# hherlyng/knp-emi-cgx

Measured on AMD Instinct MI355X. Metric: MDoF/s per implicit timestep (assembly+GMRES), higher is better.
Workload: dtype f64

## Files before the change

### include/knpemi_hip.h

```cpp
#ifndef KNPEMI_HIP_H
#define KNPEMI_HIP_H

#include <stdint.h>

#ifdef __cplusplus
extern "C" {
#endif

#define KNP_MAX_IONS 3
#define KNP_MAX_AUX 8
#define KNP_DIAG_MAX_CONSTS 64
#define KNP_MAX_PROG_REGS 48
#define KNP_MAX_AMG_LEVELS 16

#define KNP_OK 0
#define KNP_E_ARG (-1)
#define KNP_E_HIP (-2)
#define KNP_E_STATE (-3)
#define KNP_E_ALLOC (-4)
#define KNP_E_MESH (-5)

#define KNP_CONVERGED_RTOL 2
#define KNP_CONVERGED_ATOL 3
#define KNP_DIVERGED_ITS (-3)
// ... 105 lines not shown
int knp_matrix_max_abs(knp_ctx* ctx, double* out );

int knp_set_params(knp_ctx* ctx, double dt, double F, double C_M, double psi, int32_t n_ions,
                   const double* z, const double* Di, const double* De);
int knp_set_program(knp_ctx* ctx, int32_t prog_id, int32_t n_instr, const int32_t* code ,
                    int32_t n_consts, const double* consts );
const char* knp_jit_status(knp_ctx* ctx);
int knp_jit_compile_check(const int32_t* code, int32_t n_instr, const char* arch, char* log, int32_t log_cap);
int knp_host_thread_count(void);
int knp_set_program_constants(knp_ctx* ctx, int32_t prog_id, int32_t n_consts, const double* consts);
int knp_set_dirichlet(knp_ctx* ctx, int32_t n, const int32_t* dofs);
int knp_set_sources(knp_ctx* ctx, const double* const* f_i, const double* const* f_e);

int knp_assemble_matrix(knp_ctx* ctx, const knp_fields* fields);
int knp_assemble_matrix_async(knp_ctx* ctx, const knp_fields* fields);
int knp_assemble_rhs(knp_ctx* ctx, const knp_fields* fields, double* b );
int knp_assemble_precond(knp_ctx* ctx, const knp_fields* fields);
int knp_pc_set_coupled_potential(knp_ctx* ctx, int32_t on);
int knp_get_precond_phi_csr(const knp_ctx* ctx, int32_t* rowptr, int32_t* colind, double* vals);

int knp_spmv(knp_ctx* ctx, const double* x, double* y);
int knp_set_nullspace(knp_ctx* ctx, int32_t on);
int knp_project_nullspace(knp_ctx* ctx, double* v);
int knp_nullspace_test(knp_ctx* ctx, double* out_norm );
int knp_pc_setup(knp_ctx* ctx, int32_t kind);
int knp_pc_apply(knp_ctx* ctx, const double* r, double* z);
int knp_set_deflation(knp_ctx* ctx, int32_t n_modes, const int32_t* node_mode, const double* einv);
int knp_amg_reset(knp_ctx* ctx, int32_t hier, int32_t n_levels, int32_t pre_sweeps, int32_t post_sweeps, int32_t cheby_degree);
int knp_amg_set_node_fields(knp_ctx* ctx, int32_t hier, int32_t nf);
int knp_amg_set_level(knp_ctx* ctx, int32_t hier, int32_t level, int32_t n_rows, int32_t n_cols_halo,
// ... 80 lines not shown
```

### knp-emi-cgx_amd/cgx_hip/_lib.py

```python
from __future__ import annotations

import ctypes as C
import os

_HERE = os.path.dirname(os.path.abspath(__file__))
LIB_PATH = os.path.join(_HERE, "libknpemi_hip.so")

KNP_MAX_IONS = 3
KNP_MAX_AUX = 8
KNP_MAX_PROG_REGS = 48
KNP_DIAG_MAX_CONSTS = 64
KNP_SZ_COUNT = 16
(SZ_N_NODES, SZ_N_NODES_OWNED, SZ_N_DOF_LOCAL, SZ_N_DOF_OWNED, SZ_NNZ, SZ_N_PAIRS, SZ_N_CONTRIB,
 SZ_N_GAMMA_VERTS, SZ_N_GAMMA_PAIRS, SZ_NNZ_P, SZ_N_PHI_OWNED, SZ_NNZ_P_PHI, SZ_EMI_NNZ) = range(13)

PC_NONE, PC_VBJACOBI, PC_AMG, PC_AMG_BT, PC_AMG_LT = 0, 1, 2, 3, 4

OPS = dict(CONST=0, KI=1, KE=2, PHIM=3, AUX=4, X=5, ADD=6, SUB=7, MUL=8, DIV=9, NEG=10, POW=11, LN=12,
           EXP=13, SQRT=14, MAX=15, MIN=16, ABS=17, LT=18, GT=19, LE=20, GE=21, EQ=22, AND=23, OR=24,
           NOT=25, SEL=26, OUT=27, MOV=28, POWI=29)

REASONS = {2: "CONVERGED_RTOL", 3: "CONVERGED_ATOL", -3: "DIVERGED_ITS", -4: "DIVERGED_DTOL",
           -9: "DIVERGED_NANORINF", 0: "ITERATING"}

# ... 51 lines not shown
    "knp_set_nullspace": (C.c_int, [vp, C.c_int32]),
    "knp_project_nullspace": (C.c_int, [vp, vp]),
    "knp_nullspace_test": (C.c_int, [vp, f64p]),
    "knp_pc_setup": (C.c_int, [vp, C.c_int32]),
    "knp_pc_apply": (C.c_int, [vp, vp, vp]),
    "knp_set_deflation": (C.c_int, [vp, C.c_int32, i32p, f64p]),
    "knp_amg_reset": (C.c_int, [vp, C.c_int32, C.c_int32, C.c_int32, C.c_int32, C.c_int32]),
    "knp_amg_set_level": (C.c_int, [vp, C.c_int32, C.c_int32, C.c_int32, C.c_int32, i32p, i32p, f64p, f64p, C.c_double,
                                    C.c_int32, i32p, i32p, f64p, i32p, i32p, f64p]),
    "knp_amg_set_level_mode": (C.c_int, [vp, C.c_int32, C.c_int32, C.c_int32, C.c_int32]),
    "knp_amg_set_level_prolongator": (C.c_int, [vp, C.c_int32, C.c_int32, C.c_int32, C.POINTER(C.c_int32), C.POINTER(C.c_int32),
                                               C.POINTER(C.c_double)]),
    "knp_amg_set_coarse": (C.c_int, [vp, C.c_int32, C.c_int32, f64p]),
    "knp_amg_set_level_smoothed": (C.c_int, [vp, C.c_int32, C.c_int32, C.c_int32, i32p, i32p, f64p]),
    "knp_amg_set_level_coarse_fused": (C.c_int, [vp, C.c_int32, C.c_int32, C.c_int32, i32p, i32p, f64p, C.c_int32, i32p, i32p, f64p]),
    "knp_amg_set_node_fields": (C.c_int, [vp, C.c_int32, C.c_int32]),
    "knp_amg_use_native_level0": (C.c_int, [vp, C.c_int32, C.c_int32]),
    "knp_amg_set_precision": (C.c_int, [vp, C.c_int32]),
    "knp_jit_status": (C.c_char_p, [vp]),
    "knp_gmres_prepare": (C.c_int, [vp, vp]),
    "knp_jit_compile_check": (C.c_int, [C.POINTER(C.c_int32), C.c_int32, C.c_char_p, C.c_char_p, C.c_int32]),
    "knp_host_thread_count": (C.c_int, []),
    "knp_p2p_init": (C.c_int, [vp, C.c_int32, C.c_int32, C.c_double]),
    "knp_p2p_shutdown": (C.c_int, [vp]),
    "knp_p2p_plan_create": (C.c_int, [vp, C.c_int32, C.c_int64, C.c_int64, C.POINTER(C.c_int32), vp]),
    "knp_p2p_plan_connect": (C.c_int, [vp, C.c_int32, vp, C.c_int32, C.POINTER(C.c_int32), C.POINTER(C.c_int64),
                                      C.POINTER(C.c_int32), C.POINTER(C.c_int64), C.POINTER(C.c_int64), C.POINTER(C.c_int32),
                                      C.POINTER(C.c_int64)]),
    "knp_p2p_attach": (C.c_int, [vp, C.c_int32, C.c_int32, C.c_int32, C.c_int32]),
    "knp_p2p_test_halo": (C.c_int, [vp, C.c_int32, vp, C.c_int32]),
# ... 65 lines not shown
```

### knp-emi-cgx_amd/cgx_hip/backend.py

```python
from __future__ import annotations

import ctypes as C
import os

import numpy as np
import torch

from . import _lib
from ._lib import Fields, FieldsOut, KnpError, MeshDesc
from .parallel import HaloPlan, all_reduce_sum_, guarded


class _CAI:

    def __init__(self, ptr, n):
        self.__cuda_array_interface__ = {"shape": (int(n),), "typestr": "<f8", "data": (int(ptr), False),
                                         "version": 2, "strides": None}


def _f64(a):
    return a.ctypes.data_as(_lib.f64p)


def _i32(a):
# ... 373 lines not shown
            f.k_e[j] = p.wh[1][j].data_ptr()
        f.phi_i = p.wh[0][3].data_ptr()
        f.phi_e = p.wh[1][3].data_ptr()
        f.phi_m = p.phi_m_prev.data_ptr()
        self._fields_out_cache = f
        return f

    def assemble_matrix(self):
        f = self.fields()
        self.check(self.lib.knp_assemble_matrix(self.ctx, C.byref(f)))

    def assemble_matrix_async(self):
        f = self.fields()
        self.check(self.lib.knp_assemble_matrix_async(self.ctx, C.byref(f)))

    def assemble_rhs(self):
        if not getattr(self, "_programs_uploaded", False):
            self.upload_programs()
        self.refresh_program_constants()
        f = self.fields()
        self.check(self.lib.knp_assemble_rhs(self.ctx, C.byref(f), C.c_void_p(self.b.data_ptr())))

    def assemble_precond(self):
        f = self.fields()
        self.check(self.lib.knp_assemble_precond(self.ctx, C.byref(f)))

    def pack(self):
        f = self.fields_out()
        self.check(self.lib.knp_pack(self.ctx, C.byref(f), C.c_void_p(self.x.data_ptr())))

# ... 245 lines not shown
```

### knp-emi-cgx_amd/cgx_hip/problem.py

```python
from __future__ import annotations

import collections.abc
import ctypes as C
import math
import os
import pathlib
import time
from abc import ABC, abstractmethod

import numpy as np
import torch
import yaml

from . import _lib, fem
from . import mesh as meshmod
from .fem import Constant, Function, FunctionSpace
from .parallel import Comm, LocalMesh, partition_mesh


def range_constructor(loader, node):
    args = loader.construct_sequence(node)
    return list(range(*args))


# ... 533 lines not shown
            self.backend.set_sources()

    def set_initial_conditions(self):
        if self.MMS_test:
            self.print("Setting initial conditions for MMS test ...")
            dev = self.mesh.device
            as_t = lambda a: torch.as_tensor(np.array(a, dtype=np.float64, copy=True), device=dev)
            self.phi_m_prev = Function(self.V, "phi_m")
            self.phi_m_prev.x.array[:] = as_t(self._exact_nodal(self.phi_m_init))
            self.wh[0][self.N_ions].x.array[:] = as_t(self._exact_nodal(self.phi_i_init))
            self.wh[1][self.N_ions].x.array[:] = as_t(self._exact_nodal(self.phi_e_init))
            for idx, ion in enumerate(self.ion_list):
                self.wh[0][idx].x.array[:] = as_t(self._exact_nodal(ion["ki_init"]))
                self.wh[1][idx].x.array[:] = as_t(self._exact_nodal(ion["ke_init"]))
            self.print("Initial conditions set.")
            return
        if self.find_initial_conditions:
            self.find_steady_state_initial_conditions()
        else:
            self.print("Setting initial conditions from input file ...")
        ic = self.initial_conditions
        if not self.glia_flag:
            self.phi_m_init.value = ic["phi_m"] if "phi_m" in ic else ic["phi_m_n"]
            self.Na_i_init.value = ic["Na_i"] if "Na_i" in ic else ic["Na_i_n"]
            self.Na_e_init.value = ic["Na_e"]
            self.K_i_init.value = ic["K_i"] if "K_i" in ic else ic["K_i_n"]
            self.K_e_init.value = ic["K_e"]
            self.Cl_i_init.value = ic["Cl_i"] if "Cl_i" in ic else ic["Cl_i_n"]
            self.Cl_e_init.value = ic["Cl_e"]
        else:
# ... 21 lines not shown
            self.phi_m_prev.x.array[self.glia_dofs] = self.phi_m_g_init.value
            ui_p[self.N_ions].x.array[self.neuron_dofs] = self.phi_m_n_init.value
            ui_p[self.N_ions].x.array[self.glia_dofs] = self.phi_m_g_init.value
            ue_p[self.N_ions].x.array[:] = 0.0
        for idx, ion in enumerate(self.ion_list):
            if self.glia_flag:
                ui_p[idx].x.array[self.neuron_dofs] = ion["ki_init_n"].value
                ui_p[idx].x.array[self.glia_dofs] = ion["ki_init_g"].value
                ue_p[idx].x.array[:] = ion["ke_init"].value
            else:
                ui_p[idx].x.array[:] = ion["ki_init"].value
                ue_p[idx].x.array[:] = ion["ke_init"].value
                self.print(f"Initial condition for {ion['name']}_i set to {ion['ki_init'].value}")
                self.print(f"Initial condition for {ion['name']}_e set to {ion['ke_init'].value}")
        self.print("Initial conditions set.")

    def find_steady_state_initial_conditions(self):
        from .membrane_odes import ThreeCompartmentMembraneODESystem, TwoCompartmentMembraneODESystem
        self.print("Solving ODE system to find steady-state initial conditions ...")
        tic = time.perf_counter()
        self.calculate_compartment_volumes_and_surface_areas()
        areas = (self.area_g_n, self.area_g_g) if self.glia_flag else (self.area_g_n,)
        if not min(areas) > 0:
            raise RuntimeError("Steady-state initial conditions: no membrane facet carries a neuron" + (" or glia" if self.glia_flag else "")
                               + " tag (membrane tags must be the cell tags); provide 'initial_conditions' in the input file.")
        cls = ThreeCompartmentMembraneODESystem if self.glia_flag else TwoCompartmentMembraneODESystem
        odes = cls(self, plot_show=False, plot_save=False, stimulus_flag=False)
        state = None
        if self.comm.rank == 0:
            try:
# ... 199 lines not shown
```

### knp-emi-cgx_amd/cgx_hip/solver.py

```python
from __future__ import annotations

import time

import numpy as np
import torch

import os

from . import _lib, amg, dist_amg
from .ionic_models import HodgkinHuxley
from .problem import ProblemKNPEMI


class _KSPInfo:

    def __init__(self):
        self.its = 0
        self.reason = 0
        self.rnorm = 0.0

    def getIterationNumber(self):
        return self.its

    def getConvergedReason(self):
# ... 315 lines not shown
        be.set_nullspace(True)
        be.project_nullspace(be.b)
        self.print("Null space set.")

    def _matrix_scale(self):
        return self.comm.allreduce_max(self.backend.matrix_max_abs()) + 1e-300

    def _sync(self):
        torch.cuda.synchronize()

    def prepare(self):
        p = self.problem
        self.setup_breakdown = {}
        tic = time.perf_counter()
        self.setup_solver()
        self._sync()
        self.setup_breakdown["solver_setup_s"] = self.comm.allreduce_max(time.perf_counter() - tic)
        self._setup_timer = self.setup_breakdown["solver_setup_s"]
        if self.use_P_mat and self._pc_kind in (_lib.PC_AMG, _lib.PC_AMG_BT, _lib.PC_AMG_LT):
            tic = time.perf_counter()
            p.setup_preconditioner(self.use_block_Jacobi)
            self.assemble_preconditioner()
            self._sync()
            self.setup_breakdown["preconditioner_setup_s"] = self.comm.allreduce_max(time.perf_counter() - tic)
            self._setup_timer += self.setup_breakdown["preconditioner_setup_s"]
        self._n_marked = 0
        self._prepared = True

    def _resolve_timers(self):
        if not getattr(self, "_n_marked", 0):
# ... 184 lines not shown
```

### knp-emi-cgx_amd/csrc/knp_internal.hpp

```cpp
#pragma once
#include <hip/hip_runtime.h>

#include <cstdint>
#include <string>
#include <vector>

#include "knpemi_hip.h"

#define KNP_NPROF 5

struct KnpHostGraph {
    int dim = 0, nv1 = 0;
    int n_v = 0, n_v_owned = 0, n_c = 0, n_c_owned = 0, n_g = 0, n_q = 0;
    int n_nodes = 0, n_nodes_owned = 0;
    std::vector<int32_t> node_i, node_e;
    std::vector<int32_t> node_vertex;
    std::vector<uint8_t> node_side;
    std::vector<int32_t> pair_ptr;
    std::vector<int32_t> pair_col;
    std::vector<int32_t> pair_row;
    std::vector<double> pair_M, pair_K;
    std::vector<int32_t> contrib_ptr;
    std::vector<int32_t> contrib_cell;
    std::vector<double> contrib_k;
// ... 289 lines not shown
    int p2p_red = -1;
    bool hook_allreduce() const { return allreduce && p2p_red < 0; }
    int comm_rc = 0;
    int n_int = 0, n_bnd = 0;
    int32_t *d_nodes_int = nullptr, *d_nodes_bnd = nullptr;
    hipStream_t stream3 = nullptr;
    hipEvent_t ev_x = nullptr, ev_halo = nullptr;
    hipStream_t stream2 = nullptr;
    hipEvent_t ev_fork = nullptr, ev_join = nullptr;
    KnpSidePrep prep;
    bool side_ws = false;
    double *d_t2_s = nullptr, *d_w2_s = nullptr, *d_wb = nullptr, *d_partial_s = nullptr;
    hipStream_t stream_asm = nullptr;
    hipEvent_t ev_fork_asm = nullptr, ev_asm = nullptr;
    bool asm_pending = false;
    double last_bnorm = 0.0;
    int64_t n_allreduce = 0, n_halo = 0, n_readback = 0;
    int64_t n_fused_dots = 0;
    int64_t n_spmv_dots = 0;
    std::vector<hipEvent_t> tm_events;
    size_t tm_used = 0;
    KnpDiagMap diag_cells, diag_facets;
    KnpDiagMap diag_flux;
    double2* d_flux_rec = nullptr;
    KnpDiagMap diag_phim;
    int32_t* diag_code = nullptr;
    int diag_n_instr = 0, diag_n_regs = 0, diag_n_consts = 0;
    double diag_consts[KNP_DIAG_MAX_CONSTS] = {};
    bool diag_prog = false;
    KnpEmi emi;
// ... 10 lines not shown
```

### knp-emi-cgx_amd/csrc/knp_kernels.hip

```cpp
#include <hip/hip_runtime.h>
#include <hip/hip_ext.h>

#include <algorithm>
#include <cmath>
#include <cstdio>
#include <cstdlib>
#include <cstring>
#include <new>

#include "knp_internal.hpp"

#define HIPCHK(call)                                                                       \
    do {                                                                                   \
        hipError_t e_ = (call);                                                            \
        if (e_ != hipSuccess) {                                                            \
            ctx->err = std::string(#call) + ": " + hipGetErrorString(e_);                  \
            return KNP_E_HIP;                                                              \
        }                                                                                  \
    } while (0)
#define KCHK(expr)                         \
    do {                                   \
        int rc_ = (expr);                  \
        if (rc_ != KNP_OK) return rc_;     \
    } while (0)
// ... 13 lines not shown
    double dz2i[3], dz2e[3];
    double rFz[3], cmFz[3];
    double rF;
};
struct FieldPtrs {
    const double* ki[3];
    const double* ke[3];
    const double* phim;
    const double* aux[KNP_MAX_AUX];
};

static void side_discard(knp_ctx* ctx);
static DevParams make_params(const knp_ctx* ctx);
static int64_t phi_block_nnz(const knp_ctx* ctx);
static int join_asm(knp_ctx* ctx);
static bool fin_ok(const knp_ctx* ctx);
static hipEvent_t prof_event(knp_ctx* ctx);
static void free_hier(KnpAmgHier& H);
static inline int nblocks(int64_t n, int per = NT) { return (int)std::max<int64_t>(1, (n + per - 1) / per); }

__device__ __forceinline__ double wave_sum(double v) {
#pragma unroll
    for (int o = 32; o > 0; o >>= 1) v += __shfl_xor(v, o, 64);
    return v;
}
__device__ __forceinline__ double block_sum(double v, double* sm) {
    v = wave_sum(v);
    const int w = threadIdx.x >> 6, l = threadIdx.x & 63;
    __syncthreads();
    if (l == 0) sm[w] = v;
// ... 317 lines not shown
        T0 += __shfl_xor(T0, o, G);
        T1 += __shfl_xor(T1, o, G);
        T2 += __shfl_xor(T2, o, G);
    }
    if (live && selfq < 255 && (selfq & (G - 1)) == lane) emit(p0 + selfq, -T0, -T1, -T2);
}

static void launch_cell_means(knp_ctx* ctx, const FieldPtrs& f) {
    const KnpHostGraph& g = ctx->g;
    if (ctx->asm_dmax > 0)
        hipLaunchKernelGGL(k_nodal_conc, dim3(nblocks(g.n_nodes)), dim3(NT), 0, ctx->stream, g.n_nodes, ctx->d_node_vertex, ctx->d_node_side, f, ctx->d_knod);
    else
        hipLaunchKernelGGL(k_cell_means, dim3(nblocks(g.n_c)), dim3(NT), 0, ctx->stream, g.n_c, g.nv1, ctx->d_cells, ctx->d_cell_side, f, ctx->d_cbar);
}
template <bool PRECOND, bool TD_ONLY>
static void launch_assemble_nodes(knp_ctx* ctx, const DevParams& P, double* at, double* ac) {
    const KnpHostGraph& g = ctx->g;
    const int n = g.n_nodes_owned;
    if (n <= 0) return;
    if (ctx->asm_stage > 0 && ctx->d_tc_meta) {
        const int cmax = ctx->asm_stage;
        const int dmax = ctx->asm_dmax, nv1 = g.nv1;
#define KNP_ASMT2(GG, FF) hipLaunchKernelGGL((k_assemble_nodes_tr<PRECOND, TD_ONLY, GG, FF>), dim3(nblocks((int64_t)n * GG)), dim3(NT),                  \
                                        (size_t)(NT / GG) * (cmax + dmax) * 3 * sizeof(double), ctx->stream, n, P, cmax, ctx->d_pair_ptr, ctx->d_node_side, \
                                        ctx->d_pair_M, ctx->d_pair_K, ctx->d_tc_meta, ctx->d_tc_slot, ctx->d_tc_k, ctx->d_node_cell_ptr,              \
                                        ctx->d_node_cell, ctx->d_cbar, at, ac, ctx->d_pair_col, ctx->d_ncv, ctx->d_knod, dmax, nv1)
#define KNP_ASMT(GG) do { if (dmax > 0) KNP_ASMT2(GG, true); else KNP_ASMT2(GG, false); } while (0)
        switch (ctx->asm_group) {
            case 4: KNP_ASMT(4); break;
            case 8: KNP_ASMT(8); break;
            case 16: KNP_ASMT(16); break;
            default: KNP_ASMT(32); break;
        }
#undef KNP_ASMT
#undef KNP_ASMT2
        return;
    }
    if (ctx->asm_stage > 0) {
        const int cmax = ctx->asm_stage;
        const int dmax = ctx->asm_dmax, nv1 = g.nv1;
#define KNP_ASMS2(GG, FF) hipLaunchKernelGGL((k_assemble_nodes_staged<PRECOND, TD_ONLY, GG, FF>), dim3(nblocks((int64_t)n * GG)), dim3(NT),              \
                                        (size_t)(NT / GG) * (cmax + dmax) * 3 * sizeof(double), ctx->stream, n, P, cmax, ctx->d_pair_ptr, ctx->d_pair_col,  \
                                        ctx->d_node_side, ctx->d_pair_M, ctx->d_pair_K, ctx->d_contrib_ptr, ctx->d_contrib_slot, ctx->d_contrib_k, \
                                        ctx->d_node_cell_ptr, ctx->d_node_cell, ctx->d_cbar, at, ac, ctx->d_ncv, ctx->d_knod, dmax, nv1)
#define KNP_ASMS(GG) do { if (dmax > 0) KNP_ASMS2(GG, true); else KNP_ASMS2(GG, false); } while (0)
        switch (ctx->asm_group) {
            case 4: KNP_ASMS(4); break;
            case 8: KNP_ASMS(8); break;
            case 16: KNP_ASMS(16); break;
            default: KNP_ASMS(32); break;
        }
#undef KNP_ASMS
#undef KNP_ASMS2
        return;
    }
#define KNP_ASM(GG) hipLaunchKernelGGL((k_assemble_nodes<PRECOND, TD_ONLY, GG>), dim3(nblocks((int64_t)n * GG)), dim3(NT), 0, ctx->stream, n, P, ctx->d_pair_ptr, \
                                       ctx->d_pair_col, ctx->d_node_side, ctx->d_pair_M, ctx->d_pair_K, ctx->d_contrib_ptr, ctx->d_contrib_cell,       \
                                       ctx->d_contrib_k, ctx->d_cbar, at, ac)
    switch (ctx->asm_group) {
// ... 2379 lines not shown
    dev_free(ctx->d_V); dev_free(ctx->d_Z); dev_free(ctx->d_w); dev_free(ctx->d_t);
    for (auto& p : ctx->progs) { dev_free(p.d_code); dev_free(p.d_consts); if (p.h_consts) (void)hipHostFree(p.h_consts); }
    dev_free(ctx->d_prog_code); dev_free(ctx->d_prog_consts); dev_free(ctx->d_prog_len); dev_free(ctx->d_prog_nconsts);
    for (int h = 0; h < KNP_MAX_HIER; ++h) free_hier(ctx->hier[h]);
    dev_free(ctx->d_p_vals_f);
    dev_free(ctx->d_ML); dev_free(ctx->d_cc); dev_free(ctx->d_t2); dev_free(ctx->d_w2);
    dev_free(ctx->d_defl_mode); dev_free(ctx->d_defl_einv); dev_free(ctx->d_bc_dofs);
    knp_diag_free(ctx);
    knp_emi_free(ctx);
    delete ctx;
    return KNP_OK;
}

int knp_set_stream(knp_ctx* ctx, void* s) {
    CHECK_CTX(ctx);
    ctx->stream = (hipStream_t)s;
    return KNP_OK;
}
int knp_set_comm(knp_ctx* ctx, knp_halo_fn halo, knp_allreduce_fn ar, void* user) {
    CHECK_CTX(ctx);
    ctx->halo = halo; ctx->allreduce = ar; ctx->comm_user = user;
    ctx->phi_count_cached = -1;
    return KNP_OK;
}

int knp_get_sizes(const knp_ctx* ctx, int64_t* s) {
    if (!ctx || !s) return KNP_E_ARG;
    for (int i = 0; i < KNP_SZ_COUNT; ++i) s[i] = 0;
    s[KNP_SZ_N_NODES] = ctx->g.n_nodes;
    s[KNP_SZ_N_NODES_OWNED] = ctx->g.n_nodes_owned;
// ... 90 lines not shown
    HIPCHK(hipStreamSynchronize(ctx->stream));
    HIPCHK(hipMemcpy(h.data(), ctx->d_partial, h.size() * sizeof(double), hipMemcpyDeviceToHost));
    double m = 0.0;
    for (int k = 0; k < 3; ++k)
        if (len[k] > 0)
            for (int b = 0; b < RED_BLOCKS; ++b) m = std::max(m, h[(size_t)k * RED_BLOCKS + b]);
    *out = m;
    return KNP_OK;
}

int knp_set_params(knp_ctx* ctx, double dt, double F, double C_M, double psi, int32_t n_ions, const double* z,
                   const double* Di, const double* De) {
    CHECK_CTX(ctx);
    if (n_ions != 3 || !z || !Di || !De) { ctx->err = "n_ions must be 3 (Na, K, Cl; KNPEMIx_problem.py:980-981)"; return KNP_E_ARG; }
    if (!(dt > 0) || !(psi > 0) || F == 0.0) { ctx->err = "dt, psi must be positive and F non-zero"; return KNP_E_ARG; }
    ctx->dt = dt; ctx->F = F; ctx->C_M = C_M; ctx->psi = psi; ctx->n_ions = 3;
    ctx->asm_dt = -1.0;
    for (int j = 0; j < 3; ++j) {
        if (z[j] == 0.0 || !(Di[j] > 0) || !(De[j] > 0)) { ctx->err = "valence must be non-zero and diffusivities positive"; return KNP_E_ARG; }
        ctx->z[j] = z[j]; ctx->Di[j] = Di[j]; ctx->De[j] = De[j];
    }
    return KNP_OK;
}

static int validate_program(knp_ctx* ctx, int n_instr, const int32_t* code, int n_consts, int* n_regs_out) {
    int max_reg = -1;
    for (int i = 0; i < n_instr; ++i) {
        const int op = code[4 * i], d = code[4 * i + 1], a = code[4 * i + 2], b = code[4 * i + 3];
        auto regok = [&](int r) { if (r > max_reg) max_reg = r; return r >= 0 && r < KNP_MAX_PROG_REGS; };
        bool ok = true;
// ... 7 lines not shown
            case KNP_OP_MOV: case KNP_OP_POWI: ok = regok(d) && regok(a); break;
            case KNP_OP_OUT: ok = a >= 0 && a < 3 && regok(b); break;
            default: ok = (op >= KNP_OP_ADD && op <= KNP_OP_SEL) && regok(d) && regok(a) && regok(b); break;
        }
        if (!ok) { ctx->err = "invalid membrane program instruction " + std::to_string(i); return KNP_E_ARG; }
    }
    *n_regs_out = max_reg + 1;
    return KNP_OK;
}

int knp_set_program(knp_ctx* ctx, int32_t id, int32_t n_instr, const int32_t* code, int32_t n_consts, const double* consts) {
    CHECK_CTX(ctx);
    if (id < 0 || id > 4096 || n_instr < 0 || (n_instr && !code) || n_consts < 0 || (n_consts && !consts)) { ctx->err = "bad program arguments"; return KNP_E_ARG; }
    int n_regs = 0;
    KCHK(validate_program(ctx, n_instr, code, n_consts, &n_regs));
    if ((int)ctx->progs.size() <= id) ctx->progs.resize(id + 1);
    KnpProgram& p = ctx->progs[id];
    p.n_regs = n_regs;
    HIPCHK(hipStreamSynchronize(ctx->stream));
    dev_free(p.d_code); dev_free(p.d_consts);
    if (p.h_consts) { (void)hipHostFree(p.h_consts); p.h_consts = nullptr; }
    p.n_instr = n_instr; p.n_consts = n_consts;
    p.h_code.assign(code, code + (size_t)4 * n_instr);
    KCHK(dev_upload_raw(ctx, &p.d_code, code, (size_t)4 * n_instr));
    KCHK(dev_upload_raw(ctx, &p.d_consts, consts, (size_t)n_consts));
    ctx->progs_dirty = true;
    return KNP_OK;
}
int knp_set_program_constants(knp_ctx* ctx, int32_t id, int32_t n_consts, const double* consts) {
    CHECK_CTX(ctx);
// ... 28 lines not shown
    KCHK(dev_upload(ctx, &ctx->d_prog_nconsts, ncs));
    ctx->progs_dirty = false;
    knp_jit_build(ctx);
    return KNP_OK;
}

const char* knp_jit_status(knp_ctx* ctx) {
    if (!ctx) return "";
    if (ctx->progs_dirty && !ctx->progs.empty()) (void)sync_program_table(ctx);
    return ctx->jit_msg.c_str();
}

int knp_set_dirichlet(knp_ctx* ctx, int32_t n, const int32_t* dofs) {
    CHECK_CTX(ctx);
    side_discard(ctx);
    if (n < 0 || (n > 0 && !dofs)) { ctx->err = "bad Dirichlet arguments"; return KNP_E_ARG; }
    for (int i = 0; i < n; ++i)
        if (dofs[i] < 0 || dofs[i] >= ctx->n_dof_owned) { ctx->err = "Dirichlet dof out of range (owned dofs only)"; return KNP_E_ARG; }
    HIPCHK(hipStreamSynchronize(ctx->stream));
    dev_free(ctx->d_bc_dofs);
    ctx->n_bc = 0;
    if (n > 0) {
        KCHK(dev_upload_raw(ctx, &ctx->d_bc_dofs, dofs, (size_t)n));
        ctx->n_bc = n;
    }
    ctx->asm_dt = -1.0;
    return KNP_OK;
}

int knp_set_sources(knp_ctx* ctx, const double* const* fi, const double* const* fe) {
// ... 20 lines not shown
    if (ctx->pc_kind == KNP_PC_AMG || ctx->pc_kind == KNP_PC_VBJACOBI) { ctx->have_cc = false; return; }
    const KnpHostGraph& g = ctx->g;
    hipLaunchKernelGGL(k_schur_diag, dim3(nblocks(g.n_nodes_owned)), dim3(NT), 0, ctx->stream, g.n_nodes_owned, ctx->psi, ctx->z[0], ctx->z[1],
                       ctx->z[2], ctx->d_node_vertex, ctx->d_node_side, f, ctx->d_ML, ctx->d_cc);
    ctx->have_cc = true;
}

static int join_asm(knp_ctx* ctx) {
    if (ctx->asm_pending) {
        HIPCHK(hipStreamWaitEvent(ctx->stream, ctx->ev_asm, 0));
        ctx->asm_pending = false;
    }
    return KNP_OK;
}

static int assemble_matrix_on_stream(knp_ctx* ctx, const knp_fields* fields, bool with_schur_diag) {
    const KnpHostGraph& g = ctx->g;
    const DevParams P = make_params(ctx);
    FieldPtrs f = make_fields(fields);
    ProfScope ps(ctx, 3);
    launch_cell_means(ctx, f);
    const bool td_only = ctx->have_A && !ctx->asm_full && ctx->asm_dt == ctx->dt;
    if (td_only) launch_assemble_nodes<false, true>(ctx, P, ctx->d_at, ctx->d_ac);
    else launch_assemble_nodes<false, false>(ctx, P, ctx->d_at, ctx->d_ac);
    ctx->asm_dt = ctx->dt;
    if (g.n_g > 0) {
        if (g.dim == 2)
            hipLaunchKernelGGL((k_gamma_facets<2, true, false, 8, 1, NT, 1>), dim3(nblocks((int64_t)g.n_g * 8)), dim3(NT), 0, ctx->stream, g.n_g, g.n_q, P,
                               ctx->d_fv, ctx->d_fmeas, ctx->d_qp, ctx->d_qw, f, 0, ctx->d_coords, ctx->d_gamma_prog,
                               (const int32_t* const*)nullptr, (const int32_t*)nullptr, (const double* const*)nullptr,
                               (const int32_t*)nullptr, 0, 0, ctx->d_fmat, ctx->d_fvec);
        else if (gamma_many(g)) {
            hipLaunchKernelGGL((k_gamma_facets<3, true, false, 4, 9, 64, 1>), dim3((unsigned)(((int64_t)g.n_g * 4 + 63) / 64)), dim3(64), 0, ctx->stream, g.n_g, g.n_q, P,
                               ctx->d_fv, ctx->d_fmeas, ctx->d_qp, ctx->d_qw, f, 0, ctx->d_coords, ctx->d_gamma_prog,
                               (const int32_t* const*)nullptr, (const int32_t*)nullptr, (const double* const*)nullptr,
                               (const int32_t*)nullptr, 0, 0, ctx->d_fmat, ctx->d_fvec);
        }
        else
            hipLaunchKernelGGL((k_gamma_facets<3, true, false, 16, 3, 64, 2>), dim3((unsigned)(((int64_t)g.n_g * 16 + 63) / 64)), dim3(64), 0, ctx->stream, g.n_g, g.n_q, P,
// ... 12 lines not shown
    if (with_schur_diag && !ctx->prep.left()) launch_schur_diag(ctx, f);
    HIPCHK(hipGetLastError());
    ctx->have_A = true;
    if (ctx->pc_kind == KNP_PC_VBJACOBI) {
        hipLaunchKernelGGL(k_vbj_extract, dim3(nblocks(g.n_nodes_owned)), dim3(NT), 0, ctx->stream, g.n_nodes_owned,
                           ctx->d_pair_ptr, ctx->d_pair_col, ctx->d_ac, ctx->d_at, ctx->d_ax, ctx->d_node_gv, ctx->d_node_side,
                           ctx->d_gdiag, ctx->d_vbj);
        HIPCHK(hipGetLastError());
    }
    return KNP_OK;
}

int knp_assemble_matrix(knp_ctx* ctx, const knp_fields* fields) {
    CHECK_CTX(ctx);
    KCHK(check_fields(ctx, fields, false));
    KCHK(join_asm(ctx));
    return assemble_matrix_on_stream(ctx, fields, true);
}

int knp_assemble_matrix_async(knp_ctx* ctx, const knp_fields* fields) {
    CHECK_CTX(ctx);
    KCHK(check_fields(ctx, fields, false));
    KCHK(join_asm(ctx));
    static const bool off = getenv("KNP_ASM_ASYNC") && atoi(getenv("KNP_ASM_ASYNC")) == 0;
    if (off || ctx->pc_kind == KNP_PC_VBJACOBI || (ctx->prof_on & ~1) || !ctx->have_A || ctx->prep.left())
        return assemble_matrix_on_stream(ctx, fields, true);
    if (!ctx->stream_asm) {
        HIPCHK(hipStreamCreateWithFlags(&ctx->stream_asm, hipStreamNonBlocking));
        HIPCHK(hipEventCreateWithFlags(&ctx->ev_fork_asm, hipEventDisableTiming));
        HIPCHK(hipEventCreateWithFlags(&ctx->ev_asm, hipEventDisableTiming));
    }
    HIPCHK(hipEventRecord(ctx->ev_fork_asm, ctx->stream));
    HIPCHK(hipStreamWaitEvent(ctx->stream_asm, ctx->ev_fork_asm, 0));
    hipStream_t main_stream = ctx->stream;
    ctx->stream = ctx->stream_asm;
    const int rc = assemble_matrix_on_stream(ctx, fields, false);
    ctx->stream = main_stream;
    KCHK(rc);
    HIPCHK(hipEventRecord(ctx->ev_asm, ctx->stream_asm));
    ctx->asm_pending = true;
    return KNP_OK;
}

int knp_pc_set_coupled_potential(knp_ctx* ctx, int32_t on) {
    CHECK_CTX(ctx);
    side_discard(ctx);
    ctx->pc_coupled_phi = on ? 1 : 0;
    if (on && !ctx->d_px) {
        HIPCHK(hipMalloc((void**)&ctx->d_px, (size_t)std::max<int64_t>(ctx->n_gp, 1) * sizeof(double)));
        HIPCHK(hipMemset(ctx->d_px, 0, (size_t)std::max<int64_t>(ctx->n_gp, 1) * sizeof(double)));
    }
    ctx->have_P = false;
    return KNP_OK;
}
static int64_t phi_block_nnz(const knp_ctx* ctx) {
// ... 218 lines not shown
    KCHK(rc);
    if (cnt <= 0) return KNP_OK;
    const int no = ctx->g.n_nodes_owned;
    const int nb = std::min(RED_BLOCKS, nblocks(no));
    hipLaunchKernelGGL(k_phi_sum, dim3(nb), dim3(NT), 0, ctx->stream, no, v, ctx->d_partial);
    hipLaunchKernelGGL(k_reduce_partials, dim3(1), dim3(NT), 0, ctx->stream, nb, ctx->d_partial, ctx->d_red, 62, (double*)nullptr);
    KCHK(allreduce_slots(ctx, 62, 1));
    hipLaunchKernelGGL(k_phi_sub, dim3(nblocks(no)), dim3(NT), 0, ctx->stream, no, ctx->d_red + 62, 1.0 / (double)cnt, v);
    HIPCHK(hipGetLastError());
    return KNP_OK;
}
int knp_project_nullspace(knp_ctx* ctx, double* v) {
    CHECK_CTX(ctx);
    side_discard(ctx);
    if (!v) return KNP_E_ARG;
    return project_ns(ctx, v);
}

static int ensure_work(knp_ctx* ctx, int restart) {
    if (!ctx->d_w) {
        HIPCHK(hipMalloc((void**)&ctx->d_w, std::max(ctx->n_dof_local, 1) * sizeof(double)));
        HIPCHK(hipMalloc((void**)&ctx->d_t, std::max(ctx->n_dof_local, 1) * sizeof(double)));
        HIPCHK(hipMemset(ctx->d_w, 0, std::max(ctx->n_dof_local, 1) * sizeof(double)));
        HIPCHK(hipMemset(ctx->d_t, 0, std::max(ctx->n_dof_local, 1) * sizeof(double)));
    }
    if (restart > 0 && (ctx->gm_restart < restart || !ctx->d_V)) {
        HIPCHK(hipStreamSynchronize(ctx->stream));
        dev_free(ctx->d_V);
        size_t bytes = (size_t)(restart + 1) * std::max(ctx->n_dof_local, 1) * sizeof(double);
        HIPCHK(hipMalloc((void**)&ctx->d_V, bytes));
// ... 998 lines not shown
    if (n_modes == 0) return KNP_OK;
    const int no = ctx->g.n_nodes_owned;
    for (int n = 0; n < no; ++n)
        if (node_mode[n] < -1 || node_mode[n] >= n_modes) { ctx->err = "deflation mode id out of range"; return KNP_E_ARG; }
    dev_free(ctx->d_defl_mode);
    KCHK(dev_upload_raw(ctx, &ctx->d_defl_mode, node_mode, (size_t)no));
    HIPCHK(hipMemcpy(ctx->d_defl_einv, einv, (size_t)n_modes * n_modes * sizeof(double), hipMemcpyHostToDevice));
    ctx->defl_m = n_modes;
    return KNP_OK;
}

int knp_pc_apply(knp_ctx* ctx, const double* r, double* z) {
    CHECK_CTX(ctx);
    side_discard(ctx);
    if (!r || !z) return KNP_E_ARG;
    int rc;
    const int64_t cnt = ctx->ns_on ? global_phi_count(ctx, &rc) : 0;
    return pc_apply_proj(ctx, r, z, cnt);
}

#include "knp_krylov.inc"

static int out_ptrs(knp_ctx* ctx, const knp_fields_out* f, OutPtrs& o, bool need_phim) {
    if (!f) { ctx->err = "null fields"; return KNP_E_ARG; }
    for (int j = 0; j < 3; ++j) {
        if (!f->k_i[j] || !f->k_e[j]) { ctx->err = "null concentration field"; return KNP_E_ARG; }
        o.ki[j] = f->k_i[j]; o.ke[j] = f->k_e[j];
    }
    if (!f->phi_i || !f->phi_e || (need_phim && !f->phi_m)) { ctx->err = "null potential field"; return KNP_E_ARG; }
    o.phi_i = f->phi_i; o.phi_e = f->phi_e; o.phi_m = f->phi_m;
    return KNP_OK;
}
int knp_pack(knp_ctx* ctx, const knp_fields_out* f, double* x) {
    CHECK_CTX(ctx);
    if (!x) return KNP_E_ARG;
    OutPtrs o;
    KCHK(out_ptrs(ctx, f, o, false));
    hipLaunchKernelGGL(k_pack, dim3(nblocks(ctx->g.n_nodes)), dim3(NT), 0, ctx->stream, ctx->g.n_nodes, ctx->d_node_vertex,
                       ctx->d_node_side, o, x);
    HIPCHK(hipGetLastError());
    return KNP_OK;
}
int knp_unpack(knp_ctx* ctx, const double* x, const knp_fields_out* f) {
    CHECK_CTX(ctx);
    if (!x) return KNP_E_ARG;
    OutPtrs o;
    KCHK(out_ptrs(ctx, f, o, true));
    KCHK(join_asm(ctx));
    KCHK(halo_update(ctx, const_cast<double*>(x)));
    hipLaunchKernelGGL(k_unpack, dim3(nblocks(ctx->g.n_v)), dim3(NT), 0, ctx->stream, ctx->g.n_v, ctx->d_node_i, ctx->d_node_e, x, o);
    HIPCHK(hipGetLastError());
    return KNP_OK;
}
int knp_hh_update(knp_ctx* ctx, const double* phi_m, double* n, double* m, double* h, int32_t count, double dt, double phi_rest,
                  int32_t rush_larsen, int32_t substeps) {
    CHECK_CTX(ctx);
    if (!phi_m || !n || !m || !h || count < 0 || substeps < 1 || !(dt > 0)) { ctx->err = "bad hh_update arguments"; return KNP_E_ARG; }
    if (count == 0) return KNP_OK;
    ProfScope ps(ctx, 4);
    hipLaunchKernelGGL(k_hh_update, dim3(nblocks(count)), dim3(NT), 0, ctx->stream, count, phi_m, n, m, h, dt, phi_rest,
                       rush_larsen, substeps);
    HIPCHK(hipGetLastError());
    return KNP_OK;
}
int knp_l2_norms(knp_ctx* ctx, const double* phi_i, const double* phi_e, double* out) {
    CHECK_CTX(ctx);
// ... 143 lines not shown
```

### knp-emi-cgx_amd/csrc/knp_krylov.inc

```

static constexpr int GM_RES = 100, GM_EXPL = 57, GM_MAX_RESTART = GM_EXPL - 2;
static constexpr int FB_SLOT = 124;
static_assert(GM_RES + 2 <= RED_SLOTS && DEFL_SLOT0 + DEFL_MAX <= GM_RES, "reduction slot layout");
static constexpr double GM_DTOL = 1e5;

static void side_discard(knp_ctx* ctx) {
    switch (ctx->prep.kind) {
        case KnpSidePrep::NONE:
        case KnpSidePrep::LEFT_DEFERRED: break;
        default: (void)hipEventSynchronize(ctx->ev_join);
    }
    ctx->prep.kind = KnpSidePrep::NONE;
}
static int ensure_side_stream(knp_ctx* ctx) {
    if (ctx->stream2) return KNP_OK;
    HIPCHK(hipStreamCreateWithFlags(&ctx->stream2, hipStreamNonBlocking));
    HIPCHK(hipEventCreateWithFlags(&ctx->ev_fork, hipEventDisableTiming));
    HIPCHK(hipEventCreateWithFlags(&ctx->ev_join, hipEventDisableTiming));
    return KNP_OK;
}

static bool exchanges_all_native(const knp_ctx* ctx) {
    if (!ctx->p2p || ctx->p2p_fine < 0 || ctx->p2p_red < 0 || ctx->defl_m > 0) return false;
    const int nh = ctx->pc_kind == KNP_PC_AMG ? 1 : (ctx->pc_kind == KNP_PC_AMG_BT || ctx->pc_kind == KNP_PC_AMG_LT) ? 2 : 0;
// ... 182 lines not shown
    knp_ctx* ctx;
    GmLayout GL;
    double* gm;
    int n;
    int64_t ldv;
    int nb, vec_blocks;
    bool ns;
    double inv_cnt;
    double ttol, atol, dref;
};

static int krylov_begin(knp_ctx* ctx, const double* b, double* x, int32_t max_it, int32_t restart, int32_t* its, double* rnorm, int32_t* reason,
                        bool flexible, KrylovSolve* K, int64_t* cnt) {
    if (!b || !x || !its || !rnorm || !reason) return KNP_E_ARG;
    if (!ctx->have_A) { ctx->err = "matrix not assembled"; return KNP_E_STATE; }
    if (restart < 1 || restart > GM_MAX_RESTART || max_it < 0) {
        ctx->err = "restart must be in [1," + std::to_string(GM_MAX_RESTART) + "] and max_it >= 0";
        return KNP_E_ARG;
    }
    KCHK(ensure_work(ctx, restart));
    if (flexible && ctx->pc_kind != KNP_PC_NONE) KCHK(ensure_z(ctx, restart));
    prof_collect_ready(ctx);
    int rc;
    *cnt = ctx->ns_on ? global_phi_count(ctx, &rc) : 0;
    if (ctx->ns_on) KCHK(rc);
    const GmLayout GL{restart};
    if (ctx->gm_cap < GL.size()) {
        HIPCHK(hipStreamSynchronize(ctx->stream));
        dev_free(ctx->d_gm);
        HIPCHK(hipMalloc((void**)&ctx->d_gm, (size_t)GL.size() * sizeof(double)));
// ... 315 lines not shown
```

Before: 2194.

## Prefetch next-step matrix assembly on side stream right after solution unpack

After unpacking the solution into field arrays, the matrix assembly for the next timestep is launched immediately on the separate assembly stream, using the solution vector directly as nodal concentrations instead of recomputing cell means. A later async-assemble call with the same field pointers and dt becomes a no-op and is counted as a prefetch hit. Guards join the assembly stream before anything writes the solution vector, and the prefetch is invalidated whenever params, programs, Dirichlet data, the stream or initial conditions change. This hides assembly latency behind host work between steps, at the cost of extra invalidation logic and a risk of stale-data bugs if a field write is missed.

```diff
diff --git a/include/knpemi_hip.h b/include/knpemi_hip.h
--- a/include/knpemi_hip.h
+++ b/include/knpemi_hip.h
@@ -143,6 +143,9 @@
 
 int knp_assemble_matrix(knp_ctx* ctx, const knp_fields* fields);
 int knp_assemble_matrix_async(knp_ctx* ctx, const knp_fields* fields);
+int knp_set_assembly_prefetch(knp_ctx* ctx, int32_t on);
+int knp_invalidate_fields(knp_ctx* ctx);
+int knp_get_assembly_prefetch_hits(knp_ctx* ctx, int64_t* out);
 int knp_assemble_rhs(knp_ctx* ctx, const knp_fields* fields, double* b );
 int knp_assemble_precond(knp_ctx* ctx, const knp_fields* fields);
 int knp_pc_set_coupled_potential(knp_ctx* ctx, int32_t on);
diff --git a/knp-emi-cgx_amd/cgx_hip/_lib.py b/knp-emi-cgx_amd/cgx_hip/_lib.py
--- a/knp-emi-cgx_amd/cgx_hip/_lib.py
+++ b/knp-emi-cgx_amd/cgx_hip/_lib.py
@@ -89,6 +89,9 @@
     "knp_amg_set_coarse": (C.c_int, [vp, C.c_int32, C.c_int32, f64p]),
     "knp_amg_set_level_smoothed": (C.c_int, [vp, C.c_int32, C.c_int32, C.c_int32, i32p, i32p, f64p]),
     "knp_amg_set_level_coarse_fused": (C.c_int, [vp, C.c_int32, C.c_int32, C.c_int32, i32p, i32p, f64p, C.c_int32, i32p, i32p, f64p]),
+    "knp_set_assembly_prefetch": (C.c_int, [vp, C.c_int32]),
+    "knp_invalidate_fields": (C.c_int, [vp]),
+    "knp_get_assembly_prefetch_hits": (C.c_int, [vp, C.POINTER(C.c_int64)]),
     "knp_amg_set_node_fields": (C.c_int, [vp, C.c_int32, C.c_int32]),
     "knp_amg_use_native_level0": (C.c_int, [vp, C.c_int32, C.c_int32]),
     "knp_amg_set_precision": (C.c_int, [vp, C.c_int32]),
diff --git a/knp-emi-cgx_amd/cgx_hip/backend.py b/knp-emi-cgx_amd/cgx_hip/backend.py
--- a/knp-emi-cgx_amd/cgx_hip/backend.py
+++ b/knp-emi-cgx_amd/cgx_hip/backend.py
@@ -411,6 +411,19 @@
         f = self.fields()
         self.check(self.lib.knp_assemble_matrix_async(self.ctx, C.byref(f)))
 
+    def set_assembly_prefetch(self, on=True):
+        self.check(self.lib.knp_set_assembly_prefetch(self.ctx, 1 if on else 0))
+
+    def invalidate_fields(self):
+        self._fields_cache = None
+        self._fields_out_cache = None
+        self.check(self.lib.knp_invalidate_fields(self.ctx))
+
+    def assembly_prefetch_hits(self):
+        out = C.c_int64()
+        self.check(self.lib.knp_get_assembly_prefetch_hits(self.ctx, C.byref(out)))
+        return out.value
+
     def assemble_rhs(self):
         if not getattr(self, "_programs_uploaded", False):
             self.upload_programs()
diff --git a/knp-emi-cgx_amd/cgx_hip/problem.py b/knp-emi-cgx_amd/cgx_hip/problem.py
--- a/knp-emi-cgx_amd/cgx_hip/problem.py
+++ b/knp-emi-cgx_amd/cgx_hip/problem.py
@@ -571,6 +571,7 @@
                 self.wh[0][idx].x.array[:] = as_t(self._exact_nodal(ion["ki_init"]))
                 self.wh[1][idx].x.array[:] = as_t(self._exact_nodal(ion["ke_init"]))
             self.print("Initial conditions set.")
+            self._fields_rewritten()
             return
         if self.find_initial_conditions:
             self.find_steady_state_initial_conditions()
@@ -622,6 +623,12 @@
                 self.print(f"Initial condition for {ion['name']}_i set to {ion['ki_init'].value}")
                 self.print(f"Initial condition for {ion['name']}_e set to {ion['ke_init'].value}")
         self.print("Initial conditions set.")
+        self._fields_rewritten()
+
+    def _fields_rewritten(self):
+        be = getattr(self, "backend", None)
+        if be is not None and getattr(be, "ctx", None):
+            be.invalidate_fields()
 
     def find_steady_state_initial_conditions(self):
         from .membrane_odes import ThreeCompartmentMembraneODESystem, TwoCompartmentMembraneODESystem
diff --git a/knp-emi-cgx_amd/cgx_hip/solver.py b/knp-emi-cgx_amd/cgx_hip/solver.py
--- a/knp-emi-cgx_amd/cgx_hip/solver.py
+++ b/knp-emi-cgx_amd/cgx_hip/solver.py
@@ -353,6 +353,7 @@
         self.setup_breakdown = {}
         tic = time.perf_counter()
         self.setup_solver()
+        self.backend.set_assembly_prefetch(not p.MMS_test)
         self._sync()
         self.setup_breakdown["solver_setup_s"] = self.comm.allreduce_max(time.perf_counter() - tic)
         self._setup_timer = self.setup_breakdown["solver_setup_s"]
diff --git a/knp-emi-cgx_amd/csrc/knp_internal.hpp b/knp-emi-cgx_amd/csrc/knp_internal.hpp
--- a/knp-emi-cgx_amd/csrc/knp_internal.hpp
+++ b/knp-emi-cgx_amd/csrc/knp_internal.hpp
@@ -327,6 +327,16 @@
     hipStream_t stream_asm = nullptr;
     hipEvent_t ev_fork_asm = nullptr, ev_asm = nullptr;
     bool asm_pending = false;
+    int asm_prefetch = 0;
+    struct KnpPrefetch {
+        bool valid = false;
+        const double* ki[3] = {nullptr, nullptr, nullptr};
+        const double* ke[3] = {nullptr, nullptr, nullptr};
+        const double* phim = nullptr;
+        const double* x = nullptr;
+        double dt = 0.0;
+    } pf;
+    int64_t n_prefetch_hits = 0;
     double last_bnorm = 0.0;
     int64_t n_allreduce = 0, n_halo = 0, n_readback = 0;
     int64_t n_fused_dots = 0;
diff --git a/knp-emi-cgx_amd/csrc/knp_kernels.hip b/knp-emi-cgx_amd/csrc/knp_kernels.hip
--- a/knp-emi-cgx_amd/csrc/knp_kernels.hip
+++ b/knp-emi-cgx_amd/csrc/knp_kernels.hip
@@ -51,6 +51,8 @@
 static DevParams make_params(const knp_ctx* ctx);
 static int64_t phi_block_nnz(const knp_ctx* ctx);
 static int join_asm(knp_ctx* ctx);
+static int asm_invalidate(knp_ctx* ctx);
+static int asm_guard_write(knp_ctx* ctx, const double* v);
 static bool fin_ok(const knp_ctx* ctx);
 static hipEvent_t prof_event(knp_ctx* ctx);
 static void free_hier(KnpAmgHier& H);
@@ -398,17 +400,18 @@
         hipLaunchKernelGGL(k_cell_means, dim3(nblocks(g.n_c)), dim3(NT), 0, ctx->stream, g.n_c, g.nv1, ctx->d_cells, ctx->d_cell_side, f, ctx->d_cbar);
 }
 template <bool PRECOND, bool TD_ONLY>
-static void launch_assemble_nodes(knp_ctx* ctx, const DevParams& P, double* at, double* ac) {
+static void launch_assemble_nodes(knp_ctx* ctx, const DevParams& P, double* at, double* ac, const double* knod_src = nullptr) {
     const KnpHostGraph& g = ctx->g;
     const int n = g.n_nodes_owned;
     if (n <= 0) return;
+    const double* knod = knod_src ? knod_src : ctx->d_knod;
     if (ctx->asm_stage > 0 && ctx->d_tc_meta) {
         const int cmax = ctx->asm_stage;
         const int dmax = ctx->asm_dmax, nv1 = g.nv1;
 #define KNP_ASMT2(GG, FF) hipLaunchKernelGGL((k_assemble_nodes_tr<PRECOND, TD_ONLY, GG, FF>), dim3(nblocks((int64_t)n * GG)), dim3(NT),                  \
                                         (size_t)(NT / GG) * (cmax + dmax) * 3 * sizeof(double), ctx->stream, n, P, cmax, ctx->d_pair_ptr, ctx->d_node_side, \
                                         ctx->d_pair_M, ctx->d_pair_K, ctx->d_tc_meta, ctx->d_tc_slot, ctx->d_tc_k, ctx->d_node_cell_ptr,              \
-                                        ctx->d_node_cell, ctx->d_cbar, at, ac, ctx->d_pair_col, ctx->d_ncv, ctx->d_knod, dmax, nv1)
+                                        ctx->d_node_cell, ctx->d_cbar, at, ac, ctx->d_pair_col, ctx->d_ncv, knod, dmax, nv1)
 #define KNP_ASMT(GG) do { if (dmax > 0) KNP_ASMT2(GG, true); else KNP_ASMT2(GG, false); } while (0)
         switch (ctx->asm_group) {
             case 4: KNP_ASMT(4); break;
@@ -426,7 +429,7 @@
 #define KNP_ASMS2(GG, FF) hipLaunchKernelGGL((k_assemble_nodes_staged<PRECOND, TD_ONLY, GG, FF>), dim3(nblocks((int64_t)n * GG)), dim3(NT),              \
                                         (size_t)(NT / GG) * (cmax + dmax) * 3 * sizeof(double), ctx->stream, n, P, cmax, ctx->d_pair_ptr, ctx->d_pair_col,  \
                                         ctx->d_node_side, ctx->d_pair_M, ctx->d_pair_K, ctx->d_contrib_ptr, ctx->d_contrib_slot, ctx->d_contrib_k, \
-                                        ctx->d_node_cell_ptr, ctx->d_node_cell, ctx->d_cbar, at, ac, ctx->d_ncv, ctx->d_knod, dmax, nv1)
+                                        ctx->d_node_cell_ptr, ctx->d_node_cell, ctx->d_cbar, at, ac, ctx->d_ncv, knod, dmax, nv1)
 #define KNP_ASMS(GG) do { if (dmax > 0) KNP_ASMS2(GG, true); else KNP_ASMS2(GG, false); } while (0)
         switch (ctx->asm_group) {
             case 4: KNP_ASMS(4); break;
@@ -2836,6 +2839,7 @@
 
 int knp_set_stream(knp_ctx* ctx, void* s) {
     CHECK_CTX(ctx);
+    KCHK(asm_invalidate(ctx));
     ctx->stream = (hipStream_t)s;
     return KNP_OK;
 }
@@ -2956,6 +2960,7 @@
     CHECK_CTX(ctx);
     if (n_ions != 3 || !z || !Di || !De) { ctx->err = "n_ions must be 3 (Na, K, Cl; KNPEMIx_problem.py:980-981)"; return KNP_E_ARG; }
     if (!(dt > 0) || !(psi > 0) || F == 0.0) { ctx->err = "dt, psi must be positive and F non-zero"; return KNP_E_ARG; }
+    KCHK(asm_invalidate(ctx));
     ctx->dt = dt; ctx->F = F; ctx->C_M = C_M; ctx->psi = psi; ctx->n_ions = 3;
     ctx->asm_dt = -1.0;
     for (int j = 0; j < 3; ++j) {
@@ -2993,6 +2998,7 @@
     if (id < 0 || id > 4096 || n_instr < 0 || (n_instr && !code) || n_consts < 0 || (n_consts && !consts)) { ctx->err = "bad program arguments"; return KNP_E_ARG; }
     int n_regs = 0;
     KCHK(validate_program(ctx, n_instr, code, n_consts, &n_regs));
+    KCHK(asm_invalidate(ctx));
     if ((int)ctx->progs.size() <= id) ctx->progs.resize(id + 1);
     KnpProgram& p = ctx->progs[id];
     p.n_regs = n_regs;
@@ -3051,6 +3057,7 @@
 int knp_set_dirichlet(knp_ctx* ctx, int32_t n, const int32_t* dofs) {
     CHECK_CTX(ctx);
     side_discard(ctx);
+    KCHK(asm_invalidate(ctx));
     if (n < 0 || (n > 0 && !dofs)) { ctx->err = "bad Dirichlet arguments"; return KNP_E_ARG; }
     for (int i = 0; i < n; ++i)
         if (dofs[i] < 0 || dofs[i] >= ctx->n_dof_owned) { ctx->err = "Dirichlet dof out of range (owned dofs only)"; return KNP_E_ARG; }
@@ -3101,15 +3108,51 @@
     return KNP_OK;
 }
 
-static int assemble_matrix_on_stream(knp_ctx* ctx, const knp_fields* fields, bool with_schur_diag) {
+static int assemble_matrix_on_stream(knp_ctx* ctx, const FieldPtrs& f, bool with_schur_diag, const double* x_conc);
+static int asm_invalidate(knp_ctx* ctx) {
+    if (!ctx->pf.valid) return KNP_OK;
+    ctx->pf.valid = false;
+    return join_asm(ctx);
+}
+static int asm_guard_write(knp_ctx* ctx, const double* v) {
+    if (ctx->pf.valid && ctx->asm_pending && v && v == ctx->pf.x) return join_asm(ctx);
+    return KNP_OK;
+}
+static bool asm_async_excluded(const knp_ctx* ctx) {
+    static const bool off = getenv("KNP_ASM_ASYNC") && atoi(getenv("KNP_ASM_ASYNC")) == 0;
+    return off || ctx->pc_kind == KNP_PC_VBJACOBI || (ctx->prof_on & ~1) || !ctx->have_A || ctx->prep.left();
+}
+static int asm_fork(knp_ctx* ctx) {
+    if (!ctx->stream_asm) {
+        HIPCHK(hipStreamCreateWithFlags(&ctx->stream_asm, hipStreamNonBlocking));
+        HIPCHK(hipEventCreateWithFlags(&ctx->ev_fork_asm, hipEventDisableTiming));
+        HIPCHK(hipEventCreateWithFlags(&ctx->ev_asm, hipEventDisableTiming));
+    }
+    HIPCHK(hipEventRecord(ctx->ev_fork_asm, ctx->stream));
+    HIPCHK(hipStreamWaitEvent(ctx->stream_asm, ctx->ev_fork_asm, 0));
+    return KNP_OK;
+}
+static int assemble_matrix_forked(knp_ctx* ctx, const FieldPtrs& f, const double* x_conc) {
+    KCHK(asm_fork(ctx));
+    hipStream_t main_stream = ctx->stream;
+    ctx->stream = ctx->stream_asm;
+    const int rc = assemble_matrix_on_stream(ctx, f, false, x_conc);
+    ctx->stream = main_stream;
+    KCHK(rc);
+    HIPCHK(hipEventRecord(ctx->ev_asm, ctx->stream_asm));
+    ctx->asm_pending = true;
+    return KNP_OK;
+}
+
+static int assemble_matrix_on_stream(knp_ctx* ctx, const FieldPtrs& f, bool with_schur_diag, const double* x_conc) {
     const KnpHostGraph& g = ctx->g;
     const DevParams P = make_params(ctx);
-    FieldPtrs f = make_fields(fields);
     ProfScope ps(ctx, 3);
-    launch_cell_means(ctx, f);
+    const double* knod_src = (x_conc && ctx->asm_dmax > 0) ? x_conc : nullptr;
+    if (!knod_src) launch_cell_means(ctx, f);
     const bool td_only = ctx->have_A && !ctx->asm_full && ctx->asm_dt == ctx->dt;
-    if (td_only) launch_assemble_nodes<false, true>(ctx, P, ctx->d_at, ctx->d_ac);
-    else launch_assemble_nodes<false, false>(ctx, P, ctx->d_at, ctx->d_ac);
+    if (td_only) launch_assemble_nodes<false, true>(ctx, P, ctx->d_at, ctx->d_ac, knod_src);
+    else launch_assemble_nodes<false, false>(ctx, P, ctx->d_at, ctx->d_ac, knod_src);
     ctx->asm_dt = ctx->dt;
     if (g.n_g > 0) {
         if (g.dim == 2)
@@ -3152,31 +3195,42 @@
 int knp_assemble_matrix(knp_ctx* ctx, const knp_fields* fields) {
     CHECK_CTX(ctx);
     KCHK(check_fields(ctx, fields, false));
+    ctx->pf.valid = false;
     KCHK(join_asm(ctx));
-    return assemble_matrix_on_stream(ctx, fields, true);
+    return assemble_matrix_on_stream(ctx, make_fields(fields), true, nullptr);
 }
 
 int knp_assemble_matrix_async(knp_ctx* ctx, const knp_fields* fields) {
     CHECK_CTX(ctx);
     KCHK(check_fields(ctx, fields, false));
+    if (ctx->pf.valid) {
+        bool same = ctx->pf.dt == ctx->dt && ctx->pf.phim == fields->phi_m;
+        for (int j = 0; j < 3; ++j) same = same && ctx->pf.ki[j] == fields->k_i[j] && ctx->pf.ke[j] == fields->k_e[j];
+        ctx->pf.valid = false;
+        if (same && !asm_async_excluded(ctx)) {
+            ++ctx->n_prefetch_hits;
+            return KNP_OK;
+        }
+    }
     KCHK(join_asm(ctx));
-    static const bool off = getenv("KNP_ASM_ASYNC") && atoi(getenv("KNP_ASM_ASYNC")) == 0;
-    if (off || ctx->pc_kind == KNP_PC_VBJACOBI || (ctx->prof_on & ~1) || !ctx->have_A || ctx->prep.left())
-        return assemble_matrix_on_stream(ctx, fields, true);
-    if (!ctx->stream_asm) {
-        HIPCHK(hipStreamCreateWithFlags(&ctx->stream_asm, hipStreamNonBlocking));
-        HIPCHK(hipEventCreateWithFlags(&ctx->ev_fork_asm, hipEventDisableTiming));
-        HIPCHK(hipEventCreateWithFlags(&ctx->ev_asm, hipEventDisableTiming));
-    }
-    HIPCHK(hipEventRecord(ctx->ev_fork_asm, ctx->stream));
-    HIPCHK(hipStreamWaitEvent(ctx->stream_asm, ctx->ev_fork_asm, 0));
-    hipStream_t main_stream = ctx->stream;
-    ctx->stream = ctx->stream_asm;
-    const int rc = assemble_matrix_on_stream(ctx, fields, false);
-    ctx->stream = main_stream;
-    KCHK(rc);
-    HIPCHK(hipEventRecord(ctx->ev_asm, ctx->stream_asm));
-    ctx->asm_pending = true;
+    if (asm_async_excluded(ctx)) return assemble_matrix_on_stream(ctx, make_fields(fields), true, nullptr);
+    return assemble_matrix_forked(ctx, make_fields(fields), nullptr);
+}
+int knp_set_assembly_prefetch(knp_ctx* ctx, int32_t on) {
+    CHECK_CTX(ctx);
+    const bool env_off = getenv("KNP_ASM_PREFETCH") && atoi(getenv("KNP_ASM_PREFETCH")) == 0;
+    ctx->asm_prefetch = (on && !env_off) ? 1 : 0;
+    if (!ctx->asm_prefetch) KCHK(asm_invalidate(ctx));
+    return KNP_OK;
+}
+int knp_invalidate_fields(knp_ctx* ctx) {
+    CHECK_CTX(ctx);
+    return asm_invalidate(ctx);
+}
+int knp_get_assembly_prefetch_hits(knp_ctx* ctx, int64_t* out) {
+    CHECK_CTX(ctx);
+    if (!out) return KNP_E_ARG;
+    *out = ctx->n_prefetch_hits;
     return KNP_OK;
 }
 
@@ -3425,6 +3479,7 @@
     CHECK_CTX(ctx);
     side_discard(ctx);
     if (!v) return KNP_E_ARG;
+    KCHK(asm_guard_write(ctx, v));
     return project_ns(ctx, v);
 }
 
@@ -4453,6 +4508,7 @@
     CHECK_CTX(ctx);
     side_discard(ctx);
     if (!r || !z) return KNP_E_ARG;
+    KCHK(asm_guard_write(ctx, z));
     int rc;
     const int64_t cnt = ctx->ns_on ? global_phi_count(ctx, &rc) : 0;
     return pc_apply_proj(ctx, r, z, cnt);
@@ -4475,6 +4531,7 @@
     if (!x) return KNP_E_ARG;
     OutPtrs o;
     KCHK(out_ptrs(ctx, f, o, false));
+    KCHK(asm_guard_write(ctx, x));
     hipLaunchKernelGGL(k_pack, dim3(nblocks(ctx->g.n_nodes)), dim3(NT), 0, ctx->stream, ctx->g.n_nodes, ctx->d_node_vertex,
                        ctx->d_node_side, o, x);
     HIPCHK(hipGetLastError());
@@ -4489,6 +4546,20 @@
     KCHK(halo_update(ctx, const_cast<double*>(x)));
     hipLaunchKernelGGL(k_unpack, dim3(nblocks(ctx->g.n_v)), dim3(NT), 0, ctx->stream, ctx->g.n_v, ctx->d_node_i, ctx->d_node_e, x, o);
     HIPCHK(hipGetLastError());
+    ctx->pf.valid = false;
+    const bool td_only = ctx->have_A && !ctx->asm_full && ctx->asm_dt == ctx->dt;
+    if (ctx->asm_prefetch && td_only && !asm_async_excluded(ctx) && (reinterpret_cast<uintptr_t>(x) & 15) == 0) {
+        FieldPtrs fp;
+        for (int j = 0; j < 3; ++j) { fp.ki[j] = o.ki[j]; fp.ke[j] = o.ke[j]; }
+        fp.phim = o.phi_m;
+        for (int k = 0; k < KNP_MAX_AUX; ++k) fp.aux[k] = nullptr;
+        KCHK(assemble_matrix_forked(ctx, fp, x));
+        for (int j = 0; j < 3; ++j) { ctx->pf.ki[j] = o.ki[j]; ctx->pf.ke[j] = o.ke[j]; }
+        ctx->pf.phim = o.phi_m;
+        ctx->pf.dt = ctx->dt;
+        ctx->pf.x = x;
+        ctx->pf.valid = true;
+    }
     return KNP_OK;
 }
 int knp_hh_update(knp_ctx* ctx, const double* phi_m, double* n, double* m, double* h, int32_t count, double dt, double phi_rest,
diff --git a/knp-emi-cgx_amd/csrc/knp_krylov.inc b/knp-emi-cgx_amd/csrc/knp_krylov.inc
--- a/knp-emi-cgx_amd/csrc/knp_krylov.inc
+++ b/knp-emi-cgx_amd/csrc/knp_krylov.inc
@@ -220,6 +220,7 @@
                         bool flexible, KrylovSolve* K, int64_t* cnt) {
     if (!b || !x || !its || !rnorm || !reason) return KNP_E_ARG;
     if (!ctx->have_A) { ctx->err = "matrix not assembled"; return KNP_E_STATE; }
+    KCHK(asm_guard_write(ctx, x));
     if (restart < 1 || restart > GM_MAX_RESTART || max_it < 0) {
         ctx->err = "restart must be in [1," + std::to_string(GM_MAX_RESTART) + "] and max_it >= 0";
         return KNP_E_ARG;
```

Result: slower. 2163 (-1.4%).
